# briandaniel/ParallelNonlinearOptimizationLibrary

Measured on AMD Instinct MI355X. Metric: LM iters/sec at m=16384,n=2048, higher is better.
Workload: dtype f64

## Files before the change

parallelnonlinearoptimizationlibrary_amd/csrc/kernels/chol.hip:

```cpp
#include "../pnol_internal.hpp"
#include "../pnol_comm.hpp"
#include "../chol_tasks.hpp"
#include "../pnol_env.hpp"

#include <algorithm>
#include <cstdlib>
#include <type_traits>

namespace pnol {
namespace {

constexpr int NB = 64;
constexpr int kPad = 18;
constexpr int kSub = NB * kPad;
constexpr int kStage = 4 * kSub;
constexpr int kSpin = 1 << 24;
constexpr int kInfoTimeout = kCholTimeout;
typedef double d4 __attribute__((ext_vector_type(4)));

__device__ __forceinline__ double readlane_d(double v, int lane) {
    const int lo = __builtin_amdgcn_readlane(__double2loint(v), lane);
    const int hi = __builtin_amdgcn_readlane(__double2hiint(v), lane);
    return __hiloint2double(hi, lo);
}
// ... 189 lines not shown
        : "vcc", "memory");
}

template <int K, class FA, class FB>
__device__ __forceinline__ d4 mfma_blk(d4 acc, FA fa, FB fb, int lane) {
    const int i = lane & 15, kq = lane >> 4;
    double a[K / 4], b[K / 4];
#pragma unroll
    for (int q = 0; q < K / 4; ++q) {
        a[q] = fa(i, 4 * q + kq);
        b[q] = fb(i, 4 * q + kq);
    }
    d4 acc2 = {0.0, 0.0, 0.0, 0.0};
#pragma unroll
    for (int q = 0; q < K / 4; q += 2) {
        acc = __builtin_amdgcn_mfma_f64_16x16x4f64(a[q], b[q], acc, 0, 0, 0);
        acc2 = __builtin_amdgcn_mfma_f64_16x16x4f64(a[q + 1], b[q + 1], acc2, 0, 0, 0);
    }
    return acc + acc2;
}

struct DiagLds {
    double* Sl;
    double* S22;
};

__device__ __forceinline__ DiagLds diag_lds(double* smem) {
    DiagLds L;
    L.Sl = smem;
    L.S22 = smem + 64 * kS;
    return L;
}

__device__ __forceinline__ void diag_put(const DiagLds& L, int row, int col, double v) {
    if (col < kHalf) L.Sl[row * kS + col] = v;
    else if (row >= kHalf) L.S22[(row - kHalf) * kS + col - kHalf] = v;
}

struct NoEarly {
    __device__ void operator()(int, int) const {}
};

constexpr int kMW = 16;
constexpr int kBP = 18;
constexpr int kBlk = 16 * kBP;
__host__ __device__ constexpr int lblk(int ib, int jb) { return ib * (ib + 1) / 2 + jb; }
__host__ __device__ constexpr int mp_ld(int p) { return NB - kMW * p; }
__host__ __device__ constexpr int mp_base(int p) { return 1024 * p - 128 * p * (p - 1); }

struct MpLds {
    double* Sl;
    double* S22;
    double* Lc;
    double* Wb;
    double* Xs;
    double* disc;
};
__device__ __forceinline__ MpLds mp_lds(const DiagLds& L) {
    MpLds M;
    M.Sl = L.Sl;
    M.S22 = L.S22;
    M.Lc = L.S22 + kHalf * kS;
    M.Wb = M.Lc + mp_base(4);
    M.disc = M.Wb + 10 * kBlk;
    M.Xs = L.Sl;
    return M;
}
static_assert(64 * kS + kHalf * kS + mp_base(4) + 11 * kBlk <= 2 * kStage, "micro-panel factor fits the staging LDS");
static_assert(3 * kBlk <= kHalf * kS, "X hand-off blocks fit Sl rows 0..31");

__device__ __forceinline__ double w11_at(const double* W11, int r, int c) {
    return W11[lblk(r >> 4, c >> 4) * kBlk + (r & 15) * kBP + (c & 15)];
}
__device__ __forceinline__ const double* diag_w11(const DiagLds& L) { return mp_lds(L).Wb; }

__device__ __forceinline__ double* mp_s(const MpLds& M, int row, int col) {
    return col < kHalf ? M.Sl + row * kS + col : M.S22 + (row - kHalf) * kS + (col - kHalf);
}

template <int J>
struct ColBuf16 {
    static constexpr int K0 = (J + 4) & ~1, NR = K0 < kMW ? (kMW - K0) / 2 : 0;
    double2 v[NR > 0 ? NR : 1];
};

template <int J, int G>
__device__ __forceinline__ void mp_def(double (&a)[kMW], double lp2, const ColBuf16<J - 2>& cp2) {
    if constexpr (J >= 2) {
#pragma unroll
        for (int q = G; q < ColBuf16<J - 2>::NR; q += 4) {
            const int k = ColBuf16<J - 2>::K0 + 2 * q;
            if (k >= J + 2) {
                a[k] = fma(-lp2, cp2.v[q].x, a[k]);
                asm volatile("" : "+v"(a[k]));
            }
            if (k + 1 >= J + 2) {
                a[k + 1] = fma(-lp2, cp2.v[q].y, a[k + 1]);
                asm volatile("" : "+v"(a[k + 1]));
            }
        }
    }
}

#define PNOL_PIN(x) asm volatile("" : "+v"(x))
#define PNOL_SB __builtin_amdgcn_sched_barrier(0)

template <int J, int P, bool STAMP>
__device__ __forceinline__ void mp_step(double (&a)[kMW], double r, double lp1, const ColBuf16<J - 1>& cp1, double lp2,
                                        const ColBuf16<J - 2>& cp2, double* Lp, double* sb,
                                        int ss, double* __restrict__ rinv, int* cnt, int lane, bool& bad, long long* st) {
    constexpr int c = kMW * P + J, LD = mp_ld(P);
    if constexpr (STAMP && (J & 7) == 0) st[2 * P + (J >> 3)] = __builtin_amdgcn_s_memtime();
    const double l = a[J] * r;
    a[J] = l;
    double rn = 0.0;
    if constexpr (J + 1 < kMW) {
        const double piv = readlane_d(fma(-l, l, a[J + 1]), c + 1);
        double r0 = __builtin_amdgcn_rsq(piv);
        PNOL_PIN(r0);
        PNOL_SB;
        a[J + 1] = fma(-l, readlane_d(l, c + 1), a[J + 1]);
        PNOL_PIN(a[J + 1]);
        mp_def<J, 0>(a, lp2, cp2);
        PNOL_SB;
        double r2 = r0 * r0;
        PNOL_PIN(r2);
        PNOL_SB;
        if constexpr (J + 2 < kMW) {
            a[J + 2] = fma(-l, readlane_d(l, c + 2), a[J + 2]);
            PNOL_PIN(a[J + 2]);
        }
        mp_def<J, 1>(a, lp2, cp2);
        PNOL_SB;
        double e = fma(-piv, r2, 1.0);
        PNOL_PIN(e);
        PNOL_SB;
        if constexpr (J + 3 < kMW) {
            a[J + 3] = fma(-l, readlane_d(l, c + 3), a[J + 3]);
            PNOL_PIN(a[J + 3]);
        }
        mp_def<J, 2>(a, lp2, cp2);
        PNOL_SB;
        double pp = fma(e, 0.375, 0.5), re = r0 * e;
        PNOL_PIN(pp);
        PNOL_PIN(re);
        PNOL_SB;
        mp_def<J, 3>(a, lp2, cp2);
        bad |= !(piv > 0.0);
        PNOL_SB;
        rn = fma(re, pp, r0);
        PNOL_SB;
    }
    sb[J * ss] = l;
    rinv[c] = r;
    if constexpr ((J & 1) == 1) lds_signal(cnt, c + 1);
    ColBuf16<J> cv;
    if constexpr (ColBuf16<J>::NR > 0) {
#pragma unroll
        for (int q = 0; q < ColBuf16<J>::NR; ++q)
            cv.v[q] = *reinterpret_cast<const double2*>(Lp + J * LD + ColBuf16<J>::K0 + 2 * q);
    }
    asm volatile("" ::: "memory");
    PNOL_SB;
    if constexpr (J + 1 < kMW)
        mp_step<J + 1, P, STAMP>(a, rn, l, cv, lp1, cp1, Lp, sb, ss, rinv, cnt, lane, bad, st);
}

template <int P, bool STAMP>
__device__ __forceinline__ void mp_panel(const MpLds& M, double* __restrict__ rinv, int* cnt, int lane, int d,
                                         int* info, long long* st) {
    if constexpr (P == 1 || P == 2) {
        wait_lds_ge(cnt + 2, P);
        wait_lds_ge(cnt + 3, P);
    } else if constexpr (P == 3) {
        wait_lds_ge(cnt + 2, 2);
        d4 acc;
#pragma unroll
        for (int r = 0; r < 4; ++r) acc[r] = *mp_s(M, 48 + (lane >> 4) + 4 * r, 48 + (lane & 15));
        const double* Lp = M.Lc + mp_base(2);
        acc = mfma_blk<16>(acc, [&](int i, int k) { return -Lp[k * mp_ld(2) + 16 + i]; },
                           [&](int j, int k) { return Lp[k * mp_ld(2) + 16 + j]; }, lane);
#pragma unroll
        for (int r = 0; r < 4; ++r) *mp_s(M, 48 + (lane >> 4) + 4 * r, 48 + (lane & 15)) = acc[r];
    }
    double a[kMW];
    const int row = max(lane, kMW * P);
    const bool vlane = P > 0 && lane < kMW;
#pragma unroll
    for (int k = 0; k < kMW; ++k)
        a[k] = lane >= kMW * P ? *mp_s(M, row, kMW * P + k) : (vlane && k == lane ? 1.0 : 0.0);
    const double piv = readlane_d(a[0], kMW * P);
    bool bad = !(piv > 0.0);
    const ColBuf16<-1> n1{};
    const ColBuf16<-2> n2{};
    double* const Lp = M.Lc + mp_base(P);
    double* const sb = (P == 0 || lane >= kMW * P) ? Lp + (lane - kMW * P)
                                                   : (vlane ? M.Wb + lblk(P, P) * kBlk + lane : M.disc + lane);
    const int ss = (P == 0 || lane >= kMW * P) ? mp_ld(P) : (vlane ? kBP : 0);
    mp_step<0, P, STAMP>(a, rsqrt_nr(piv), 0.0, n1, 0.0, n2, Lp, sb, ss, rinv, cnt, lane, bad, st);
    if (bad && lane == 0) atomicCAS(info, 0, d * NB + kMW * P + 1);
}

__device__ __forceinline__ void blk_put(double* __restrict__ B, const d4& acc, int lane) {
#pragma unroll
    for (int r = 0; r < 4; ++r) B[((lane >> 4) + 4 * r) * kBP + (lane & 15)] = acc[r];
}

template <int OW>
__device__ __forceinline__ void mp_owner(const MpLds& M, int* cnt, int lane, const double* __restrict__ Lsrc, int kb0) {
    const int frow = lane & 15, fk = lane >> 4;
    auto lld = [&](d4& acc, int ib, int q) {
#pragma unroll
        for (int r = 0; r < 4; ++r) acc[r] = *mp_s(M, 16 * ib + (lane >> 4) + 4 * r, 16 * q + (lane & 15));
        if (Lsrc && kb0 < 4) {
            double fa[4][4], fb[4][4];
#pragma unroll
            for (int kb = 0; kb < 4; ++kb)
                if (kb >= kb0)
#pragma unroll
                    for (int kk = 0; kk < 4; ++kk) {
                        fa[kb][kk] = -Lsrc[kb * kSub + (ib * 16 + frow) * kPad + kk * 4 + fk];
                        fb[kb][kk] = Lsrc[kb * kSub + (q * 16 + frow) * kPad + kk * 4 + fk];
                    }
#pragma unroll
            for (int kb = 0; kb < 4; ++kb)
                if (kb >= kb0)
#pragma unroll
                    for (int kk = 0; kk < 4; ++kk)
                        acc = __builtin_amdgcn_mfma_f64_16x16x4f64(fa[kb][kk], fb[kb][kk], acc, 0, 0, 0);
        }
    };
    auto upd = [&](d4& acc, int ib, int q, auto pc, int g) {
        constexpr int P = decltype(pc)::value, LD = mp_ld(P);
        const double* Lp = M.Lc + mp_base(P);
        const double x = -Lp[(4 * g + fk) * LD + 16 * ib - kMW * P + frow];
        const double y = Lp[(4 * g + fk) * LD + 16 * q - kMW * P + frow];
        acc = __builtin_amdgcn_mfma_f64_16x16x4f64(x, y, acc, 0, 0, 0);
    };
    auto put = [&](const d4& acc, int ib, int q) {
#pragma unroll
        for (int r = 0; r < 4; ++r) *mp_s(M, 16 * ib + (lane >> 4) + 4 * r, 16 * q + (lane & 15)) = acc[r];
    };
    constexpr int NA = OW == 2 ? 2 : 1;
    const int ia[2] = {OW == 2 ? 1 : 2, 3};
    d4 a[NA];
#pragma unroll
    for (int b = 0; b < NA; ++b) lld(a[b], ia[b], 1);
#pragma unroll
    for (int g = 0; g < 4; ++g) {
        wait_lds_ge(cnt, 4 * g + 4);
#pragma unroll
        for (int b = 0; b < NA; ++b) upd(a[b], ia[b], 1, std::integral_constant<int, 0>(), g);
    }
#pragma unroll
    for (int b = 0; b < NA; ++b) put(a[b], ia[b], 1);
    lds_signal(cnt + OW, 1);
    constexpr int NB2 = OW == 2 ? 1 : 2;
    const int ibb[2] = {3, OW == 2 ? 3 : 2}, qb[2] = {OW == 2 ? 3 : 2, 2};
    d4 c[NB2];
#pragma unroll
    for (int b = 0; b < NB2; ++b) lld(c[b], ibb[b], qb[b]);
#pragma unroll
    for (int g = 0; g < 4; ++g)
#pragma unroll
        for (int b = 0; b < NB2; ++b) upd(c[b], ibb[b], qb[b], std::integral_constant<int, 0>(), g);
#pragma unroll
    for (int g = 0; g < 4; ++g) {
        wait_lds_ge(cnt, kMW + 4 * g + 4);
#pragma unroll
        for (int b = 0; b < NB2; ++b) upd(c[b], ibb[b], qb[b], std::integral_constant<int, 1>(), g);
    }
#pragma unroll
    for (int b = 0; b < NB2; ++b) put(c[b], ibb[b], qb[b]);
    lds_signal(cnt + OW, 2);
}

template <int P>
__device__ __forceinline__ void mp_inverse(const MpLds& M, const double* __restrict__ rinv, const int* cnt, int lane) {
    constexpr int LD = mp_ld(P);
    const double* Lp = M.Lc + mp_base(P);
    double y[kMW];
#pragma unroll
    for (int k = 0; k < kMW; ++k) y[k] = (k == lane) ? 1.0 : 0.0;
    auto step = [&](auto jc) {
        constexpr int J = decltype(jc)::value, K0 = J, NR = (kMW - K0) / 2;
        wait_lds_ge(cnt, kMW * P + J + 2);
        double2 c0[NR], c1[NR];
#pragma unroll
        for (int q = 0; q < NR; ++q) {
            c0[q] = *reinterpret_cast<const double2*>(Lp + J * LD + K0 + 2 * q);
            c1[q] = *reinterpret_cast<const double2*>(Lp + (J + 1) * LD + K0 + 2 * q);
        }
        const double r0 = rinv[kMW * P + J], r1 = rinv[kMW * P + J + 1];
        __builtin_amdgcn_sched_barrier(0);
        const double w0 = y[J] * r0;
        y[J] = w0;
        y[J + 1] = fma(-c0[0].y, w0, y[J + 1]);
        const double w1 = y[J + 1] * r1;
        y[J + 1] = w1;
#pragma unroll
        for (int q = 1; q < NR; ++q) {
            const int k = K0 + 2 * q;
            y[k] = fma(-c0[q].x, w0, y[k]);
            y[k + 1] = fma(-c0[q].y, w0, y[k + 1]);
            y[k] = fma(-c1[q].x, w1, y[k]);
            y[k + 1] = fma(-c1[q].y, w1, y[k + 1]);
        }
        asm volatile("" ::: "memory");
        __builtin_amdgcn_sched_barrier(0);
    };
    step(std::integral_constant<int, 0>());
    step(std::integral_constant<int, 2>());
    step(std::integral_constant<int, 4>());
    step(std::integral_constant<int, 6>());
    step(std::integral_constant<int, 8>());
    step(std::integral_constant<int, 10>());
    step(std::integral_constant<int, 12>());
    step(std::integral_constant<int, 14>());
    double* dst = (lane < kMW ? M.Wb + lblk(P, P) * kBlk : M.disc) + (lane & 15);
#pragma unroll
    for (int k = 0; k < kMW; ++k) dst[k * kBP] = y[k];
}

template <int I, int K, int J>
__device__ __forceinline__ d4 mp_lw(d4 acc, const MpLds& M, int lane) {
    const double* Lp = M.Lc + mp_base(K);
    const double* Wk = M.Wb + lblk(K, J) * kBlk;
    return mfma_blk<16>(acc, [&](int i, int k) { return Lp[k * mp_ld(K) + 16 * (I - K) + i]; },
                        [&](int j, int k) { return Wk[k * kBP + j]; }, lane);
}
template <int I, int J>
__device__ __forceinline__ void mp_vx(const MpLds& M, const double* __restrict__ X, int lane) {
    const double* Vi = M.Wb + lblk(I, I) * kBlk;
    d4 acc = {0.0, 0.0, 0.0, 0.0};
    acc = mfma_blk<16>(acc, [&](int i, int k) { return -Vi[i * kBP + k]; }, [&](int j, int k) { return X[k * kBP + j]; },
                       lane);
    blk_put(M.Wb + lblk(I, J) * kBlk, acc, lane);
}

template <bool SC1, int IB>
__device__ __forceinline__ void mp_w_rows(const MpLds& M, double* __restrict__ Wd, int lane) {
    const int jb = lane >> 4, c = lane & 15;
    double v[16];
#pragma unroll
    for (int q = 0; q < 16; ++q) v[q] = jb <= IB ? M.Wb[lblk(IB, jb <= IB ? jb : 0) * kBlk + q * kBP + c] : 0.0;
#pragma unroll
    for (int q = 0; q < 16; ++q) stg<SC1>(Wd + (16 * IB + q) * NB + lane, v[q]);
}

template <bool STAMP = false, bool SC1 = false, class EARLY = NoEarly>
__device__ __forceinline__ void factor_diag16(const DiagLds& L, double* __restrict__ rinv, int* cnt,
                                              double* __restrict__ Wd, int d, int* info, long long* st = nullptr,
                                              const EARLY& early = EARLY(), double* __restrict__ Wst = nullptr,
                                              const double* __restrict__ Lsrc = nullptr, int kb0 = 4) {
    const int t = threadIdx.x, wave = __builtin_amdgcn_readfirstlane(t >> 6), lane = t & 63;
    const MpLds M = mp_lds(L);
    if (wave == 0) {
        mp_panel<0, STAMP>(M, rinv, cnt, lane, d, info, st);
        mp_panel<1, STAMP>(M, rinv, cnt, lane, d, info, st);
        mp_panel<2, STAMP>(M, rinv, cnt, lane, d, info, st);
        mp_panel<3, STAMP>(M, rinv, cnt, lane, d, info, st);
        if constexpr (STAMP) st[8] = __builtin_amdgcn_s_memtime();
        wait_lds_ge(cnt + 4, 1);
        mp_vx<3, 0>(M, M.Xs, lane);
        mp_vx<3, 1>(M, M.Xs + kBlk, lane);
        if constexpr (STAMP) st[9] = __builtin_amdgcn_s_memtime();
    } else if (wave == 1) {
        const d4 z = {0.0, 0.0, 0.0, 0.0};
        mp_inverse<0>(M, rinv, cnt, lane);
        d4 x10 = mp_lw<1, 0, 0>(z, M, lane), x20 = mp_lw<2, 0, 0>(z, M, lane), x30 = mp_lw<3, 0, 0>(z, M, lane);
        wait_lds_ge(cnt, 2 * kMW);
        if constexpr (STAMP) st[10] = __builtin_amdgcn_s_memtime();
        blk_put(M.Xs, x10, lane);
        mp_vx<1, 0>(M, M.Xs, lane);
        lds_signal(cnt + 1, 1);
        mp_w_rows<SC1, 0>(M, Wd, lane);
        mp_w_rows<SC1, 1>(M, Wd, lane);
        d4 x21 = mp_lw<2, 1, 1>(z, M, lane), x31 = mp_lw<3, 1, 1>(z, M, lane);
        x20 = mp_lw<2, 1, 0>(x20, M, lane);
        x30 = mp_lw<3, 1, 0>(x30, M, lane);
        wait_lds_ge(cnt, 3 * kMW);
        if constexpr (STAMP) st[11] = __builtin_amdgcn_s_memtime();
        blk_put(M.Xs, x20, lane);
        blk_put(M.Xs + kBlk, x21, lane);
        mp_vx<2, 0>(M, M.Xs, lane);
        mp_vx<2, 1>(M, M.Xs + kBlk, lane);
        d4 x32 = mp_lw<3, 2, 2>(z, M, lane);
        x30 = mp_lw<3, 2, 0>(x30, M, lane);
        x31 = mp_lw<3, 2, 1>(x31, M, lane);
        blk_put(M.Xs, x30, lane);
        blk_put(M.Xs + kBlk, x31, lane);
        blk_put(M.Xs + 2 * kBlk, x32, lane);
        lds_signal(cnt + 4, 1);
        mp_w_rows<SC1, 2>(M, Wd, lane);
        wait_lds_ge(cnt, 4 * kMW);
        if constexpr (STAMP) st[12] = __builtin_amdgcn_s_memtime();
        mp_vx<3, 2>(M, M.Xs + 2 * kBlk, lane);
    } else {
        if (wave == 2) mp_owner<2>(M, cnt, lane, Lsrc, kb0);
        else mp_owner<3>(M, cnt, lane, Lsrc, kb0);
        wait_lds_ge(cnt + 1, 1);
        early(wave, lane);
    }
    __syncthreads();
    if constexpr (STAMP) if (wave == 0) st[13] = __builtin_amdgcn_s_memtime();
    {
        const int jb = lane >> 4, c = lane & 15;
        double v[16];
#pragma unroll
        for (int q = 0; q < 16; ++q) {
            const int ib = wave;
            v[q] = jb <= ib ? M.Wb[lblk(ib, jb <= ib ? jb : 0) * kBlk + q * kBP + c] : 0.0;
        }
        if (wave == 3)
#pragma unroll
            for (int q = 0; q < 16; ++q) stg<SC1>(Wd + (16 * wave + q) * NB + lane, v[q]);
        if (Wst) {
            __syncthreads();
#pragma unroll
            for (int q = 0; q < 16; ++q) Wst[jb * kSub + (16 * wave + q) * kPad + c] = v[q];
        }
    }
}

template <bool STAMP = false, bool SC1 = false, class EARLY = NoEarly>
__device__ __forceinline__ void factor_diag(const DiagLds& L, double* __restrict__ rinv, int* cnt,
                                            double* __restrict__ Wd, int d, int* info, long long* st = nullptr,
                                            const EARLY& early = EARLY(), double* __restrict__ Wst = nullptr,
                                            const double* __restrict__ Lsrc = nullptr, int kb0 = 4) {
    factor_diag16<STAMP, SC1, EARLY>(L, rinv, cnt, Wd, d, info, st, early, Wst, Lsrc, kb0);
}

__device__ __forceinline__ void diag_l_strip(d4 (&acc)[4], const double* __restrict__ X, const double* __restrict__ Y,
                                             int w, int lane) {
    const int frow = lane & 15, fk = lane >> 4;
#pragma unroll
    for (int jb = 0; jb < 4; ++jb) acc[jb] = d4{0.0, 0.0, 0.0, 0.0};
    double a[4][4], b[10][4];
#pragma unroll
    for (int kb = 0; kb < 4; ++kb)
#pragma unroll
        for (int kk = 0; kk < 4; ++kk) {
            a[kb][kk] = X[kb * kSub + (w * 16 + frow) * kPad + kk * 4 + fk];
#pragma unroll
            for (int jb = kb; jb < 4; ++jb)
                b[kb * 4 - kb * (kb - 1) / 2 + jb - kb][kk] = Y[kb * kSub + (jb * 16 + frow) * kPad + kk * 4 + fk];
        }
#pragma unroll
    for (int kb = 0; kb < 4; ++kb)
#pragma unroll
        for (int kk = 0; kk < 4; ++kk)
#pragma unroll
            for (int jb = kb; jb < 4; ++jb)
                acc[jb] = __builtin_amdgcn_mfma_f64_16x16x4f64(a[kb][kk], b[kb * 4 - kb * (kb - 1) / 2 + jb - kb][kk], acc[jb],
                                                               0, 0, 0);
}

__device__ __forceinline__ void diag_strip_to_stage(const d4 (&acc)[4], double* __restrict__ X, int w, int lane) {
#pragma unroll
    for (int jb = 0; jb < 4; ++jb)
#pragma unroll
        for (int r = 0; r < 4; ++r) X[jb * kSub + (w * 16 + (lane >> 4) + 4 * r) * kPad + (lane & 15)] = acc[jb][r];
}

__device__ __forceinline__ void diag_l_blocks(d4 (&acc)[2], const double* __restrict__ X, const double* __restrict__ Y,
                                              int s, int j0, int j1, int lane) {
    const int frow = lane & 15, fk = lane >> 4;
    acc[0] = acc[1] = d4{0.0, 0.0, 0.0, 0.0};
#pragma unroll
    for (int kb = 0; kb < 4; ++kb)
#pragma unroll
        for (int kk = 0; kk < 4; ++kk) {
            const double a = X[kb * kSub + (s * 16 + frow) * kPad + kk * 4 + fk];
            if (kb <= j0)
                acc[0] = __builtin_amdgcn_mfma_f64_16x16x4f64(a, Y[kb * kSub + (j0 * 16 + frow) * kPad + kk * 4 + fk],
                                                              acc[0], 0, 0, 0);
            if (kb <= j1)
                acc[1] = __builtin_amdgcn_mfma_f64_16x16x4f64(a, Y[kb * kSub + (j1 * 16 + frow) * kPad + kk * 4 + fk],
                                                              acc[1], 0, 0, 0);
        }
}

__device__ __forceinline__ void mfma_xyt_half(d4 (&acc)[2], const double* __restrict__ X, const double* __restrict__ Y,
                                              int h, int w, int lane) {
    const int frow = lane & 15, fk = lane >> 4;
#pragma unroll
    for (int sub = 0; sub < 4; ++sub)
#pragma unroll
        for (int kk = 0; kk < 4; ++kk) {
            const double b = Y[sub * kSub + (w * 16 + frow) * kPad + kk * 4 + fk];
#pragma unroll
            for (int mi = 0; mi < 2; ++mi) {
                const double a = -X[sub * kSub + ((2 * h + mi) * 16 + frow) * kPad + kk * 4 + fk];
                acc[mi] = __builtin_amdgcn_mfma_f64_16x16x4f64(a, b, acc[mi], 0, 0, 0);
            }
        }
}

template <bool SC1 = false>
__device__ __forceinline__ void strip_store(const d4 (&acc)[4], double* __restrict__ Lm, long ldp, int r0, int c0, int w,
                                            int lane) {
#pragma unroll
    for (int jb = 0; jb < 4; ++jb)
#pragma unroll
        for (int r = 0; r < 4; ++r)
            stg<SC1>(Lm + (long)(r0 + w * 16 + (lane >> 4) + 4 * r) * ldp + c0 + jb * 16 + (lane & 15), acc[jb][r]);
}
__device__ __forceinline__ void strip_to_rows(const d4 (&acc)[4], double* __restrict__ S, int w, int lane) {
#pragma unroll
    for (int jb = 0; jb < 4; ++jb)
#pragma unroll
        for (int r = 0; r < 4; ++r) S[(w * 16 + (lane >> 4) + 4 * r) * (NB + 1) + jb * 16 + (lane & 15)] = acc[jb][r];
}

__device__ __forceinline__ int diag_blk(int w, int s) {
    constexpr int tab[4][3] = {{(3 << 2) | 0, (3 << 2) | 1, 0}, {(3 << 2) | 2, (3 << 2) | 3, (1 << 2) | 0},
                               {(2 << 2) | 0, (2 << 2) | 1, -1}, {(2 << 2) | 2, (1 << 2) | 1, -1}};
    return tab[w][s];
}
__device__ __forceinline__ int diag_blk_def(int w, int s) {
    constexpr int tab[4][3] = {{0, (3 << 2) | 1, (1 << 2) | 1}, {(1 << 2) | 0, (3 << 2) | 2, (3 << 2) | 3},
                               {(2 << 2) | 0, (2 << 2) | 1, -1}, {(3 << 2) | 0, (2 << 2) | 2, -1}};
    return tab[w][s];
}

#ifdef PNOL_CHOL_TIMELINE
__device__ unsigned long long g_chol_tl[64 * 3 * 2];
__device__ unsigned long long g_chol_clk[64 * 8];
__device__ unsigned long long g_chol_crit[64 * 8];
__device__ unsigned long long g_chol_la[64 * 4];
#define PNOL_LA_STAMP(d, i) \
    if (threadIdx.x == 128 && (d) < 64) g_chol_la[4 * (d) + (i)] = __builtin_amdgcn_s_memtime();
#define PNOL_CRIT(k, i) \
    if (threadIdx.x == 0 && (k) >= 0 && (k) < 64) g_chol_crit[8 * (k) + (i)] = __builtin_amdgcn_s_memrealtime();
#define PNOL_CRIT_IF(c, k, i) \
    if (c) { PNOL_CRIT(k, i) }
#define PNOL_CHOL_CLK_PUT(k, i, v) \
    if (threadIdx.x == 0 && (k) + 1 < 64) g_chol_clk[8 * ((k) + 1) + (i)] = (v);
#define PNOL_CHOL_STAMP(k, i) PNOL_CHOL_CLK_PUT(k, i, __builtin_amdgcn_s_memtime())
__device__ __forceinline__ void chol_tl_mark(int k, int cls, unsigned long long t0) {
    if (threadIdx.x == 0 && k + 1 < 64) {
        const unsigned long long t1 = __builtin_amdgcn_s_memrealtime();
        atomicMin(&g_chol_tl[((k + 1) * 3 + cls) * 2], t0);
        atomicMax(&g_chol_tl[((k + 1) * 3 + cls) * 2 + 1], t1);
    }
}
#define PNOL_TL_BEGIN() const unsigned long long tl0_ = __builtin_amdgcn_s_memrealtime();
#define PNOL_TL_BEGIN_CLK() PNOL_TL_BEGIN() const unsigned long long ck0_ = __builtin_amdgcn_s_memtime();
#define PNOL_TL_MARK(k, cls) chol_tl_mark(k, cls, tl0_);
#define PNOL_TL_BARRIER() __syncthreads();
#define PNOL_TL_DIAG_END(k) PNOL_TL_MARK(k, 0) PNOL_CHOL_CLK_PUT(k, 0, ck0_) PNOL_CHOL_STAMP(k, 7)
#else
#define PNOL_CHOL_CLK_PUT(k, i, v)
#define PNOL_CHOL_STAMP(k, i)
#define PNOL_CRIT(k, i)
#define PNOL_CRIT_IF(c, k, i)
#define PNOL_LA_STAMP(d, i)
#define PNOL_TL_BEGIN()
#define PNOL_TL_BEGIN_CLK()
#define PNOL_TL_MARK(k, cls)
#define PNOL_TL_BARRIER()
#define PNOL_TL_DIAG_END(k)
#endif
#ifdef PNOL_CHOL_TASKTRACE
__device__ unsigned long long g_chol_tasks[16384 * 4];
#define PNOL_TASK_T0(g) const unsigned long long tt0_ = __builtin_amdgcn_s_memrealtime(); const int tg_ = (g);
#define PNOL_TASK_READY() const unsigned long long tt1_ = __builtin_amdgcn_s_memrealtime();
#define PNOL_TASK_END(k, kind)                                                                         \
    if (threadIdx.x == 0 && tg_ < 16384) {                                                              \
        g_chol_tasks[4 * tg_] = tt0_;                                                                  \
        g_chol_tasks[4 * tg_ + 1] = tt1_;                                                              \
        g_chol_tasks[4 * tg_ + 2] = __builtin_amdgcn_s_memrealtime();                                  \
        g_chol_tasks[4 * tg_ + 3] = ((unsigned long long)(k) << 8) | (unsigned long long)(kind);       \
    }
#else
#define PNOL_TASK_T0(g)
#define PNOL_TASK_READY()
#define PNOL_TASK_END(k, kind)
#endif

template <bool SC1 = false>
__device__ __forceinline__ void diag_prepare(const double* __restrict__ P, long ldp, const double* __restrict__ W,
                                             int k, double* __restrict__ X, double* __restrict__ Y, const DiagLds& L,
// ... 455 lines not shown
    const double* jp = nullptr;
    double* rhs = nullptr;
    const double* packed = nullptr;
    long slot = 0;
    int tpr = 1;
    const double* rhs_in = nullptr;
    bool preloaded = false;
    int order = 1;
    bool selfl = true;
    bool split = true;
    bool rowmajor = true;
};

template <int SUB>
__device__ __forceinline__ void red_pair(const double* __restrict__ p, long off, int sub, double& vx, double& vy) {
    constexpr long E = 128L * 128L;
    double lx[8], ly[8];
#pragma unroll
    for (int s = 0; s < 8; ++s) {
        double ax = 0.0, ay = 0.0;
#pragma unroll
        for (int u = 0; u < (SUB > 0 ? SUB : sub); ++u) {
            const double2 w = *reinterpret_cast<const double2*>(p + (long)(s * sub + u) * E + off);
            ax += w.x;
            ay += w.y;
        }
        lx[s] = ax;
        ly[s] = ay;
    }
    vx = ((lx[0] + lx[1]) + (lx[2] + lx[3])) + ((lx[4] + lx[5]) + (lx[6] + lx[7]));
    vy = ((ly[0] + ly[1]) + (ly[2] + ly[3])) + ((ly[4] + ly[5]) + (ly[6] + ly[7]));
}

__device__ void red_task(int u, const RedArgs& red, double* __restrict__ P, long ldp, int T, double* __restrict__ bv,
                         const PersistWords& pw, int* __restrict__ info) {
    const int t = threadIdx.x;
    if (u == 0 && red.rhs_in) {
        for (int e = t; e < red.n; e += 256) stg<true>(bv + e, red.rhs_in[e]);
        asm volatile("s_waitcnt vmcnt(0)" ::: "memory");
        __syncthreads();
        for (int i = t; i < T; i += 256) __hip_atomic_store(pw.bcnt + i, 0, __ATOMIC_RELAXED, __HIP_MEMORY_SCOPE_AGENT);
        return;
    }
    if (u == 0) {
        for (int e = t; e < red.n; e += 256) {
            double l[8];
#pragma unroll
            for (int s = 0; s < 8; ++s) l[s] = 0.0 + red.jp[(long)s * red.n + e];
            const double v = ((l[0] + l[1]) + (l[2] + l[3])) + ((l[4] + l[5]) + (l[6] + l[7]));
            red.rhs[e] = v;
            stg<true>(bv + e, v);
        }
        asm volatile("s_waitcnt vmcnt(0)" ::: "memory");
        __syncthreads();
        for (int i = t; i < T; i += 256) __hip_atomic_store(pw.bcnt + i, 0, __ATOMIC_RELAXED, __HIP_MEMORY_SCOPE_AGENT);
        return;
    }
    int r = u - 1, J = 0;
    while (r >= T - J) {
        r -= T - J;
        ++J;
    }
    const int I = J + r, ti = I >> 1, tj = J >> 1;
    const long tt = (long)ti * (ti + 1) / 2 + tj;
    const double* p = red.part ? red.part + tt * 8 * red.sub * (128L * 128L) : nullptr;
    const double* pk = red.packed ? red.packed + (tt / red.tpr) * red.slot + (tt % red.tpr) * (128L * 128L) : nullptr;
    const double scale = 1 + red.lambda;
    auto pairs = [&](auto SUBC) {
        constexpr int S = decltype(SUBC)::value;
        for (int q0 = t; q0 < NB * NB / 2; q0 += 512) {
            double v[2][2];
#pragma unroll
            for (int w = 0; w < 2; ++w) {
                const int q = q0 + 256 * w, rr = q >> 5, c = 2 * (q & 31);
                const long off = (long)(64 * (I & 1) + rr) * 128 + 64 * (J & 1) + c;
                if (pk) {
                    const double2 pv = *reinterpret_cast<const double2*>(pk + off);
                    v[w][0] = pv.x;
                    v[w][1] = pv.y;
                } else {
                    red_pair<S>(p, off, red.sub, v[w][0], v[w][1]);
                }
            }
#pragma unroll
            for (int w = 0; w < 2; ++w) {
                const int q = q0 + 256 * w, rr = q >> 5, c = 2 * (q & 31);
                const int i = I * NB + rr;
#pragma unroll
                for (int h = 0; h < 2; ++h) {
                    const int j = J * NB + c + h;
                    if (i >= red.n || j >= red.n || j > i) continue;
                    stg<true>(P + (long)i * ldp + j, i == j ? scale * v[w][h] : v[w][h]);
                    if (j < i && I == J) stg<true>(P + (long)j * ldp + i, v[w][h]);
                }
            }
        }
    };
    if (red.sub == 2) pairs(std::integral_constant<int, 2>{});
    else pairs(std::integral_constant<int, 0>{});
    publish(pw.ver + I * T + J, 0);
}


__device__ __forceinline__ bool wait_w(const PersistWords pw, int k, bool w0_prep, int* info) {
    return (k == 0 && w0_prep) || spin_ge(pw.wdone + k, 1, info);
}

__device__ __forceinline__ bool selfl_wait_tiles(int T, const PersistWords pw, int i, int j, int k, int& ok_sh,
                                                 int* info) {
    if (threadIdx.x == 0)
        ok_sh = spin_all<3>({pw.ver + i * T + j, pw.ver + i * T + k, pw.ver + j * T + k}, {k, k, k}, info);
    __syncthreads();
    return ok_sh;
}
__device__ __forceinline__ bool selfl_stage(const double* __restrict__ P, long ldp, const double* __restrict__ W,
                                            const PersistWords pw, int i, int j, int k, bool w0_prep,
                                            double* __restrict__ X, double* __restrict__ Y, double* __restrict__ Z,
                                            int& ok_sh, int* info, [[maybe_unused]] bool stamp) {
    const int k0 = k * NB;
    stage_tile<true>(X, P, ldp, i * NB, k0);
    if (i != j) stage_tile<true>(Z, P, ldp, j * NB, k0);
    if (threadIdx.x == 0) ok_sh = wait_w(pw, k, w0_prep, info);
    __syncthreads();
    if (!ok_sh) return false;
    PNOL_CRIT_IF(stamp, k, 5)
    stage_tile<true>(Y, W + (long)k * NB * NB, NB, 0, 0);
    __syncthreads();
    return true;
}

__global__ __launch_bounds__(256, 1) void k_chol_persist(double* __restrict__ P, double* __restrict__ Lm, long ldp,
                                                      int T, double* __restrict__ W, double* __restrict__ bv,
                                                      double* __restrict__ zv, int* __restrict__ flags, int ntasks,
                                                      int* __restrict__ info, int lookahead,
                                                      const RedArgs red) {
    __shared__ __attribute__((aligned(16))) double smem[2 * kStage];
    __shared__ __attribute__((aligned(16))) double pfx[kStage];
    __shared__ __attribute__((aligned(16))) double pll[2 * kSub];
    __shared__ __attribute__((aligned(16))) double pfc[kLowerBlks * 256];
    __shared__ double rinv[NB];
    __shared__ double zsh[NB];
    __shared__ int cnt[6];
    __shared__ int ew[4];
    __shared__ int task_sh, ok_sh;
    const int t = threadIdx.x, lane = t & 63, wave = __builtin_amdgcn_readfirstlane(t >> 6), wr = wave >> 1, wc = wave & 1;
    const PersistWords pw = persist_words(flags, T);
    double* X = smem;
    double* Y = smem + kStage;
    const bool w0_prep = !red.part && !red.packed && !red.preloaded, smode = !w0_prep;

    if (blockIdx.x == 0) {
        const EarlyLds E{pfx, pll, pfc, ew};
        if (t < 4) ew[t] = 0;
        for (int d = smode ? 0 : 1; d < T; ++d) {
            const int k = d - 1;
            PNOL_TL_BEGIN_CLK()
            if (t == 0) {
                const bool ok = __hip_atomic_load(info, __ATOMIC_RELAXED, __HIP_MEMORY_SCOPE_AGENT) == 0 &&
                                (d == 0 ? spin_ge(pw.ver, 0, info)
                                        : spin_all<2>({pw.ver + d * T + k, pw.ver + d * T + d}, {k, k}, info));
                ok_sh = ok;
            }
            __syncthreads();
            if (!ok_sh) return;
            PNOL_CHOL_STAMP(k, 5)
            const DiagLds L = diag_lds(smem);
            const bool pre = lookahead && ew[0] == 1;
            const bool staged = lookahead && ew[0] == 3;
            PNOL_CHOL_CLK_PUT(k, 6, pre ? 1 : (staged ? 2 : 0))
            if (d == 0) {
                const int row = t >> 2, c0 = (t & 3) * 16;
                double v[16];
#pragma unroll
                for (int q = 0; q < 16; ++q) v[q] = ldg<true>(P + (long)row * ldp + c0 + q);
#pragma unroll
                for (int q = 0; q < 16; ++q) diag_put(L, row, c0 + q, v[q]);
            } else if (pre) {
                late_prepare(E, Y, L, wave, lane, true);
            } else {
                diag_prepare<true>(P, ldp, W, k, X, Y, L, wave, lane, d > 1 || smode, pfx, staged ? pfx : nullptr,
                                   staged ? pfc : nullptr);
            }
            if (t < 6) cnt[t] = 0;
            if (t < 4) ew[t] = 0;
            __syncthreads();
            PNOL_CHOL_STAMP(k, 3)
            const int kb0 = d == 0 ? 4 : (pre ? 2 : 0);
            if (lookahead)
                factor_diag<false, true, EarlyNext>(L, rinv, cnt, W + (long)d * NB * NB, d, info, nullptr,
                                                    EarlyNext{P, ldp, T, d, pw.ver, diag_w11(L), cnt, lookahead, E}, Y,
                                                    pfx, kb0);
            else
                factor_diag<false, true>(L, rinv, cnt, W + (long)d * NB * NB, d, info, nullptr, NoEarly(), Y, pfx, kb0);
            PNOL_CHOL_STAMP(k, 4)
            publish(pw.wdone + d, 1);
            PNOL_CRIT(d, 0)
            PNOL_TL_DIAG_END(k)
        }
        return;
    }

    const int nred = (red.part || red.packed) ? chol_reduce_task_count(T) : 0;
    const bool split = red.selfl && red.split;
    const int order = chol_claim_order(red.order, (int)gridDim.x - 1, split);
    int pre = -1;
    for (;;) {
        if (t == 0) {
            task_sh = pre >= 0 ? pre : atomicAdd(pw.counter, 1);
            pre = -1;
        }
        __syncthreads();
        int g = task_sh;
        __syncthreads();
        if (g >= nred + ntasks) return;
        if (g < nred) {
            red_task(g, red, P, ldp, T, bv, pw, info);
            continue;
        }
        g -= nred;
        PNOL_TASK_T0(g)
        const Task tk = task_of(g, T, order, split, red.rowmajor);
        const int k = tk.k;
        const int k0 = k * NB;
        if (tk.j < 0) {
            const int i = tk.i, i0 = i * NB;
            PNOL_TL_BEGIN()
            PNOL_CRIT_IF(i == k + 2, k, 1)
            if (t == 0) ok_sh = spin_all<3>({pw.ver + i * T + k, pw.bcnt + k, pw.bcnt + i}, {k, k, k}, info);
            __syncthreads();
            if (!ok_sh) return;
            stage_tile<true>(X, P, ldp, i0, k0);
            if (t == 0) {
                ok_sh = wait_w(pw, k, w0_prep, info);
                PNOL_CRIT_IF(i == k + 2, k, 2)
            }
            __syncthreads();
            if (!ok_sh) return;
            stage_tile<true>(Y, W + (long)k * NB * NB, NB, 0, 0);
            __syncthreads();
            PNOL_TASK_READY()
            d4 acc[4];
            diag_l_strip(acc, X, Y, wave, lane);
            strip_store<true>(acc, Lm, ldp, i0, k0, wave, lane);
            publish(pw.lcnt + i, k + 1);
            PNOL_CRIT_IF(i == k + 2, k, 3)
            PNOL_CRIT_IF(i == k + 1, k, 7)
            strip_to_rows(acc, X, wave, lane);
            if (t < NB) {
                double s = 0.0;
#pragma unroll 16
                for (int j = 0; j < NB; ++j) s = fma(Y[(j >> 4) * kSub + t * kPad + (j & 15)], ldg<true>(bv + k0 + j), s);
                zsh[t] = s;
            }
            __syncthreads();
            if (t < NB) {
                double s = 0.0;
#pragma unroll 16
                for (int j = 0; j < NB; ++j) s = fma(X[t * (NB + 1) + j], zsh[j], s);
                stg<true>(bv + i0 + t, ldg<true>(bv + i0 + t) - s);
                if (i == k + 1) stg<true>(zv + k0 + t, zsh[t]);
            }
            publish_claim(pw.bcnt + i, k + 1, pw.counter, pre);
            PNOL_TASK_END(k, 0)
            PNOL_TL_MARK(k, 1)
            continue;
        }
        const int i = tk.i, j = tk.j;
        PNOL_TL_BEGIN()
        [[maybe_unused]] const bool crit = i == k + 2 && j == k + 1;
        PNOL_CRIT_IF(crit, k, 4)
        if (tk.h >= 0) {
            const int h = tk.h, w = wave;
            double* Z = pfx;
            d4 acc[2];
            if (!selfl_wait_tiles(T, pw, i, j, k, ok_sh, info)) return;
#pragma unroll
            for (int mi = 0; mi < 2; ++mi)
#pragma unroll
                for (int r = 0; r < 4; ++r)
                    acc[mi][r] = ldg<true>(P + (long)(i * NB + (2 * h + mi) * 16 + (lane >> 4) + 4 * r) * ldp +
                                           j * NB + w * 16 + (lane & 15));
            if (!selfl_stage(P, ldp, W, pw, i, j, k, w0_prep, X, Y, Z, ok_sh, info, crit && h == 0)) return;
            PNOL_TASK_READY()
            if (i != j) {
                const int s = 2 * h + (w >> 1), j0 = (w & 1) ? 1 : 0, j1 = (w & 1) ? 2 : 3;
                d4 lh[2], lj[4];
                diag_l_blocks(lh, X, Y, s, j0, j1, lane);
                diag_l_strip(lj, Z, Y, w, lane);
                __syncthreads();
#pragma unroll
                for (int r = 0; r < 4; ++r) {
                    X[j0 * kSub + (s * 16 + (lane >> 4) + 4 * r) * kPad + (lane & 15)] = lh[0][r];
                    X[j1 * kSub + (s * 16 + (lane >> 4) + 4 * r) * kPad + (lane & 15)] = lh[1][r];
                }
                diag_strip_to_stage(lj, Z, w, lane);
            } else {
                d4 li[4];
                diag_l_strip(li, X, Y, w, lane);
                __syncthreads();
                diag_strip_to_stage(li, X, w, lane);
            }
            __syncthreads();
            mfma_xyt_half(acc, X, i != j ? Z : X, h, w, lane);
#pragma unroll
            for (int mi = 0; mi < 2; ++mi)
#pragma unroll
                for (int r = 0; r < 4; ++r)
                    stg<true>(P + (long)(i * NB + (2 * h + mi) * 16 + (lane >> 4) + 4 * r) * ldp + j * NB + w * 16 +
                                  (lane & 15),
                              acc[mi][r]);
            publish_half_claim(pw.half + i * T + j, pw.ver + i * T + j, k + 1, pw.counter, pre);
            PNOL_TASK_END(k, 2)
            PNOL_CRIT_IF(crit, k, 6)
            PNOL_TL_MARK(k, 2)
            continue;
        }
        if (red.selfl && i == k + 2 && j >= k + 1) {
            double* Z = pfx;
            d4 acc[2][2];
            if (!selfl_wait_tiles(T, pw, i, j, k, ok_sh, info)) return;
            acc_load<true>(acc, P, ldp, i * NB, j * NB, wr, wc, lane);
            if (!selfl_stage(P, ldp, W, pw, i, j, k, w0_prep, X, Y, Z, ok_sh, info, crit)) return;
            PNOL_TASK_READY()
            d4 li[4], lj[4];
            diag_l_strip(li, X, Y, wave, lane);
            if (i != j) diag_l_strip(lj, Z, Y, wave, lane);
            __syncthreads();
            diag_strip_to_stage(li, X, wave, lane);
            if (i != j) diag_strip_to_stage(lj, Z, wave, lane);
            __syncthreads();
            mfma_xyt<true>(acc, X, i != j ? Z : X, wr, wc, lane);
            acc_store<true>(acc, P, ldp, i * NB, j * NB, wr, wc, lane);
            publish_claim(pw.ver + i * T + j, k + 1, pw.counter, pre);
            PNOL_TASK_END(k, 3)
            PNOL_CRIT_IF(crit, k, 6)
            PNOL_TL_MARK(k, 2)
            continue;
        }
        if (t == 0) {
            ok_sh = ready_all<3>({pw.ver + i * T + j, pw.lcnt + i, pw.lcnt + j}, {k, k + 1, k + 1})
                        ? 2
                        : spin_ge(pw.ver + i * T + j, k, info);
        }
        __syncthreads();
        const int st0 = ok_sh;
        if (!st0) return;
        d4 acc[2][2];
// ... 332 lines not shown
```

Baseline: 314.0.

## Trim diagonal-factor sync: fewer LDS signals, direct W row-3 stores, prefetched readiness

Panels other than the first now write rinv only for P==0 and raise the LDS counter every fourth column instead of every second. Wave 0 and wave 1 write the last W block-row straight to global memory from the MFMA accumulators, replacing a separate pass after the barrier. The diagonal block loop samples info and the next step's version flags right after factoring and skips the spin when they are already satisfied. A ROLES/POLL template hook (defaulted on) is added for experiments that replace polling with fixed sleeps. The aim is to cut handshake, barrier and spin latency on the serial diagonal critical path, at the cost of coarser-grained signalling and readiness checks that may use stale flags.

Result: no change. 316.1, median of 2 (+0.7%).

```diff
diff --git a/parallelnonlinearoptimizationlibrary_amd/csrc/kernels/chol.hip b/parallelnonlinearoptimizationlibrary_amd/csrc/kernels/chol.hip
--- a/parallelnonlinearoptimizationlibrary_amd/csrc/kernels/chol.hip
+++ b/parallelnonlinearoptimizationlibrary_amd/csrc/kernels/chol.hip
@@ -365,8 +365,8 @@
         PNOL_SB;
     }
     sb[J * ss] = l;
-    rinv[c] = r;
-    if constexpr ((J & 1) == 1) lds_signal(cnt, c + 1);
+    if constexpr (P == 0) rinv[c] = r;
+    if constexpr ((J & 1) == 1 && (P == 0 || (J & 3) == 3)) lds_signal(cnt, c + 1);
     ColBuf16<J> cv;
     if constexpr (ColBuf16<J>::NR > 0) {
 #pragma unroll
@@ -419,7 +419,7 @@
     for (int r = 0; r < 4; ++r) B[((lane >> 4) + 4 * r) * kBP + (lane & 15)] = acc[r];
 }
 
-template <int OW>
+template <int OW, bool POLL = true>
 __device__ __forceinline__ void mp_owner(const MpLds& M, int* cnt, int lane, const double* __restrict__ Lsrc, int kb0) {
     const int frow = lane & 15, fk = lane >> 4;
     auto lld = [&](d4& acc, int ib, int q) {
@@ -461,7 +461,8 @@
     for (int b = 0; b < NA; ++b) lld(a[b], ia[b], 1);
 #pragma unroll
     for (int g = 0; g < 4; ++g) {
-        wait_lds_ge(cnt, 4 * g + 4);
+        if constexpr (POLL) wait_lds_ge(cnt, 4 * g + 4);
+        else __builtin_amdgcn_s_sleep(15);
 #pragma unroll
         for (int b = 0; b < NA; ++b) upd(a[b], ia[b], 1, std::integral_constant<int, 0>(), g);
     }
@@ -479,7 +480,8 @@
         for (int b = 0; b < NB2; ++b) upd(c[b], ibb[b], qb[b], std::integral_constant<int, 0>(), g);
 #pragma unroll
     for (int g = 0; g < 4; ++g) {
-        wait_lds_ge(cnt, kMW + 4 * g + 4);
+        if constexpr (POLL) wait_lds_ge(cnt, kMW + 4 * g + 4);
+        else __builtin_amdgcn_s_sleep(15);
 #pragma unroll
         for (int b = 0; b < NB2; ++b) upd(c[b], ibb[b], qb[b], std::integral_constant<int, 1>(), g);
     }
@@ -543,12 +545,18 @@
                         [&](int j, int k) { return Wk[k * kBP + j]; }, lane);
 }
 template <int I, int J>
-__device__ __forceinline__ void mp_vx(const MpLds& M, const double* __restrict__ X, int lane) {
+__device__ __forceinline__ d4 mp_vx(const MpLds& M, const double* __restrict__ X, int lane) {
     const double* Vi = M.Wb + lblk(I, I) * kBlk;
     d4 acc = {0.0, 0.0, 0.0, 0.0};
     acc = mfma_blk<16>(acc, [&](int i, int k) { return -Vi[i * kBP + k]; }, [&](int j, int k) { return X[k * kBP + j]; },
                        lane);
     blk_put(M.Wb + lblk(I, J) * kBlk, acc, lane);
+    return acc;
+}
+template <bool SC1>
+__device__ __forceinline__ void w3_store(double* __restrict__ Wd, int J, const d4& acc, int lane) {
+#pragma unroll
+    for (int r = 0; r < 4; ++r) stg<SC1>(Wd + (48 + (lane >> 4) + 4 * r) * NB + 16 * J + (lane & 15), acc[r]);
 }
 
 template <bool SC1, int IB>
@@ -561,7 +569,7 @@
     for (int q = 0; q < 16; ++q) stg<SC1>(Wd + (16 * IB + q) * NB + lane, v[q]);
 }
 
-template <bool STAMP = false, bool SC1 = false, class EARLY = NoEarly>
+template <bool STAMP = false, bool SC1 = false, class EARLY = NoEarly, int ROLES = 15>
 __device__ __forceinline__ void factor_diag16(const DiagLds& L, double* __restrict__ rinv, int* cnt,
                                               double* __restrict__ Wd, int d, int* info, long long* st = nullptr,
                                               const EARLY& early = EARLY(), double* __restrict__ Wst = nullptr,
@@ -575,10 +583,10 @@
         mp_panel<3, STAMP>(M, rinv, cnt, lane, d, info, st);
         if constexpr (STAMP) st[8] = __builtin_amdgcn_s_memtime();
         wait_lds_ge(cnt + 4, 1);
-        mp_vx<3, 0>(M, M.Xs, lane);
-        mp_vx<3, 1>(M, M.Xs + kBlk, lane);
+        w3_store<SC1>(Wd, 0, mp_vx<3, 0>(M, M.Xs, lane), lane);
+        w3_store<SC1>(Wd, 1, mp_vx<3, 1>(M, M.Xs + kBlk, lane), lane);
         if constexpr (STAMP) st[9] = __builtin_amdgcn_s_memtime();
-    } else if (wave == 1) {
+    } else if (wave == 1 && (ROLES & 2)) {
         const d4 z = {0.0, 0.0, 0.0, 0.0};
         mp_inverse<0>(M, rinv, cnt, lane);
         d4 x10 = mp_lw<1, 0, 0>(z, M, lane), x20 = mp_lw<2, 0, 0>(z, M, lane), x30 = mp_lw<3, 0, 0>(z, M, lane);
@@ -608,16 +616,20 @@
         mp_w_rows<SC1, 2>(M, Wd, lane);
         wait_lds_ge(cnt, 4 * kMW);
         if constexpr (STAMP) st[12] = __builtin_amdgcn_s_memtime();
-        mp_vx<3, 2>(M, M.Xs + 2 * kBlk, lane);
-    } else {
-        if (wave == 2) mp_owner<2>(M, cnt, lane, Lsrc, kb0);
-        else mp_owner<3>(M, cnt, lane, Lsrc, kb0);
+        w3_store<SC1>(Wd, 2, mp_vx<3, 2>(M, M.Xs + 2 * kBlk, lane), lane);
+        d4 w33;
+#pragma unroll
+        for (int r = 0; r < 4; ++r) w33[r] = M.Wb[lblk(3, 3) * kBlk + ((lane >> 4) + 4 * r) * kBP + (lane & 15)];
+        w3_store<SC1>(Wd, 3, w33, lane);
+    } else if (wave >= 2 && (ROLES & 4)) {
+        if (wave == 2) mp_owner<2, (ROLES & 8) != 0>(M, cnt, lane, Lsrc, kb0);
+        else mp_owner<3, (ROLES & 8) != 0>(M, cnt, lane, Lsrc, kb0);
         wait_lds_ge(cnt + 1, 1);
         early(wave, lane);
     }
     __syncthreads();
     if constexpr (STAMP) if (wave == 0) st[13] = __builtin_amdgcn_s_memtime();
-    {
+    if (Wst) {
         const int jb = lane >> 4, c = lane & 15;
         double v[16];
 #pragma unroll
@@ -625,23 +637,18 @@
             const int ib = wave;
             v[q] = jb <= ib ? M.Wb[lblk(ib, jb <= ib ? jb : 0) * kBlk + q * kBP + c] : 0.0;
         }
-        if (wave == 3)
-#pragma unroll
-            for (int q = 0; q < 16; ++q) stg<SC1>(Wd + (16 * wave + q) * NB + lane, v[q]);
-        if (Wst) {
-            __syncthreads();
-#pragma unroll
-            for (int q = 0; q < 16; ++q) Wst[jb * kSub + (16 * wave + q) * kPad + c] = v[q];
-        }
-    }
-}
-
-template <bool STAMP = false, bool SC1 = false, class EARLY = NoEarly>
+        __syncthreads();
+#pragma unroll
+        for (int q = 0; q < 16; ++q) Wst[jb * kSub + (16 * wave + q) * kPad + c] = v[q];
+    }
+}
+
+template <bool STAMP = false, bool SC1 = false, class EARLY = NoEarly, int ROLES = 15>
 __device__ __forceinline__ void factor_diag(const DiagLds& L, double* __restrict__ rinv, int* cnt,
                                             double* __restrict__ Wd, int d, int* info, long long* st = nullptr,
                                             const EARLY& early = EARLY(), double* __restrict__ Wst = nullptr,
                                             const double* __restrict__ Lsrc = nullptr, int kb0 = 4) {
-    factor_diag16<STAMP, SC1, EARLY>(L, rinv, cnt, Wd, d, info, st, early, Wst, Lsrc, kb0);
+    factor_diag16<STAMP, SC1, EARLY, ROLES>(L, rinv, cnt, Wd, d, info, st, early, Wst, Lsrc, kb0);
 }
 
 __device__ __forceinline__ void diag_l_strip(d4 (&acc)[4], const double* __restrict__ X, const double* __restrict__ Y,
@@ -1403,13 +1410,18 @@
     if (blockIdx.x == 0) {
         const EarlyLds E{pfx, pll, pfc, ew};
         if (t < 4) ew[t] = 0;
+        int nx_info = 0, nx_v0 = -1, nx_v1 = -1;
+        bool nx_have = false, nx_lds = false;
         for (int d = smode ? 0 : 1; d < T; ++d) {
             const int k = d - 1;
             PNOL_TL_BEGIN_CLK()
             if (t == 0) {
-                const bool ok = __hip_atomic_load(info, __ATOMIC_RELAXED, __HIP_MEMORY_SCOPE_AGENT) == 0 &&
-                                (d == 0 ? spin_ge(pw.ver, 0, info)
-                                        : spin_all<2>({pw.ver + d * T + k, pw.ver + d * T + d}, {k, k}, info));
+                const int inf = nx_have ? nx_info : __hip_atomic_load(info, __ATOMIC_RELAXED, __HIP_MEMORY_SCOPE_AGENT);
+                const bool nx_ready = nx_have && (nx_lds || (nx_v0 >= k && nx_v1 >= k));
+                const bool ok = inf == 0 &&
+                                (nx_ready ||
+                                 (d == 0 ? spin_ge(pw.ver, 0, info)
+                                         : spin_all<2>({pw.ver + d * T + k, pw.ver + d * T + d}, {k, k}, info)));
                 ok_sh = ok;
             }
             __syncthreads();
@@ -1444,6 +1456,16 @@
             else
                 factor_diag<false, true>(L, rinv, cnt, W + (long)d * NB * NB, d, info, nullptr, NoEarly(), Y, pfx, kb0);
             PNOL_CHOL_STAMP(k, 4)
+            if (t == 0 && d + 1 < T) {
+                const int dn = d + 1;
+                nx_have = true;
+                nx_info = __hip_atomic_load(info, __ATOMIC_RELAXED, __HIP_MEMORY_SCOPE_AGENT);
+                nx_lds = lookahead && (ew[0] == 1 || ew[0] == 3);
+                if (!nx_lds) {
+                    nx_v0 = __hip_atomic_load(pw.ver + dn * T + d, __ATOMIC_RELAXED, __HIP_MEMORY_SCOPE_AGENT);
+                    nx_v1 = __hip_atomic_load(pw.ver + dn * T + dn, __ATOMIC_RELAXED, __HIP_MEMORY_SCOPE_AGENT);
+                }
+            }
             publish(pw.wdone + d, 1);
             PNOL_CRIT(d, 0)
             PNOL_TL_DIAG_END(k)
```
